# Animesh005/Torus-FHE

Measured on AMD Instinct MI355X. Metric: bootstrapped gates/sec (NAND, N=1024), higher is better.
Workload: dtype f64

## Files before the change

### torus-fhe_amd/csrc/thfhe_common.h

```cpp
#ifndef THFHE_COMMON_H
#define THFHE_COMMON_H

#include <hip/hip_runtime.h>

#include <type_traits>

#include "../../include/thfhe_hip.h"
#include "thfhe_lane.h"

namespace thfhe {

constexpr int kOpIdentity = 100;

int thfhe_fail(int code, const char *msg);
int thfhe_fail_hip(hipError_t e, const char *what);

inline int ilog2(int x) {
    int l = 0;
    while ((1 << l) < x) l++;
    return l;
}

inline int lut_validate(const thfhe_lut_spec *sp, const void *tv, int n_luts, const int32_t *lut_index, const int32_t *in0, const int32_t *in1,
                        const int32_t *in2, const int32_t *out, size_t count, int max_luts = 1024) {
// ... 5 lines not shown
    if (count > (size_t)INT32_MAX / 16) return thfhe_fail(THFHE_E_INVALID, "count too large");
    if (lut_index)
        for (size_t g = 0; g < count; g++)
            if (lut_index[g] < 0 || lut_index[g] >= n_luts) return thfhe_fail(THFHE_E_INVALID, "lut_index out of range (0 .. n_luts-1)");
    return THFHE_OK;
}

inline int lut_spec_check(const thfhe_lut_spec &sp) {
    if (sp.n_inputs < 1 || sp.n_inputs > 3) return thfhe_fail(THFHE_E_INVALID, "lut spec: n_inputs must be 1, 2 or 3");
    if (sp.theta != 1 && sp.theta != 2 && sp.theta != 4) return thfhe_fail(THFHE_E_INVALID, "lut spec: theta must be 1, 2 or 4");
    return THFHE_OK;
}

#define THFHE_HIP(expr)                                                    \
    do {                                                                   \
        hipError_t thfhe_e_ = (expr);                                      \
        if (thfhe_e_ != hipSuccess) return ::thfhe::thfhe_fail_hip(thfhe_e_, #expr); \
    } while (0)

template <int Max, int V = 1, class F>
int with_static_int(int v, const char *unsupported, F &&f) {
    if constexpr (V > Max) return thfhe_fail(THFHE_E_UNSUPPORTED, unsupported);
    else if (v == V) {
        f(std::integral_constant<int, V>{});
        return THFHE_OK;
    } else return with_static_int<Max, V + 1>(v, unsupported, f);
}
constexpr const char *kBadL = "decomposition length l must be 1..4";

inline int kernel_name_result(int len, int need) {
    return need < len ? THFHE_OK : thfhe_fail(THFHE_E_INVALID, "buffer too short for the kernel name");
}

#if defined(__HIPCC__)
#ifdef THFHE_STAMPS
#define THFHE_STAMP_STORAGE __device__ unsigned long long g_stamps[8 * 2048 * 8];
#define STAMP_DECL unsigned long long st_acc[6] = {0, 0, 0, 0, 0, 0}, st_t = __builtin_amdgcn_s_memtime()
#define STAMP(slot)                                              \
    do {                                                         \
        unsigned long long now_ = __builtin_amdgcn_s_memtime();  \
        st_acc[slot] += now_ - st_t;                             \
        st_t = now_;                                             \
    } while (0)
#define STAMP_FLUSH(wg, wave)                                                                                  \
    do {                                                                                                       \
        if (lane == 0 && (wg) < 2048)                                                                          \
            for (int q_ = 0; q_ < 6; q_++) g_stamps[(((size_t)(wg)) * 8 + (wave)) * 8 + q_] = st_acc[q_];       \
    } while (0)
#else
#define THFHE_STAMP_STORAGE
#define STAMP_DECL
#define STAMP(slot)
#define STAMP_FLUSH(wg, wave)
#endif


__device__ __forceinline__ void wave_sync() {
    __builtin_amdgcn_fence(__ATOMIC_RELEASE, "wavefront", "local");
    __builtin_amdgcn_wave_barrier();
    __builtin_amdgcn_fence(__ATOMIC_ACQUIRE, "wavefront", "local");
}

__device__ __forceinline__ int opaque_lane(int lane) {
    asm volatile("" : "+v"(lane));
    return lane;
}
typedef const int32_t __attribute__((address_space(4))) *uniform_i32_ptr;
__device__ __forceinline__ uniform_i32_ptr as_uniform(const int32_t *p) { return (uniform_i32_ptr)(size_t)p; }

template <int IMM = 0>
__device__ __forceinline__ void ring_dma(uint64_t gbase_uniform, uint32_t lane_byte_off, uint32_t lds_byte_off) {
    static_assert(IMM >= 0 && IMM < 4096, "immediate offset of a global instruction");
    asm volatile("s_nop 0\n\tglobal_load_lds_dwordx4 %0, %1 offset:%3" ::"v"(lane_byte_off), "s"(gbase_uniform), "{m0}"(lds_byte_off), "n"(IMM) : "memory");
}
template <int VM>
__device__ __forceinline__ void ring_barrier() {
    asm volatile("s_waitcnt vmcnt(%0) lgkmcnt(0)\n\ts_barrier" ::"n"(VM) : "memory");
}
__device__ __forceinline__ void wave_fft_fwd_s(int lane, cplx (&z)[8], cplx *xb, const cplx *T1, const W64 &w) {
    wave_sync();
    fwds_seg1(lane, z, xb, T1);
    wave_sync();
    fwds_seg2_ld(lane, z, xb);
    fwds_seg2_st(lane, z, xb, w);
    wave_sync();
    fwds_seg3(lane, z, xb);
}
__device__ __forceinline__ void wave_fft_inv_s(int lane, cplx (&z)[8], cplx *xb, const cplx *T1, const W64 &w) {
    wave_sync();
    invs_seg1(lane, z, xb, w);
    wave_sync();
    invs_seg2_ld(lane, z, xb);
    invs_seg2_st(lane, z, xb);
    wave_sync();
    invs_seg3(lane, z, xb, T1);
}
template <bool KEEP64 = false>
__device__ __forceinline__ void wave_transpose_hi3(cplx (&z)[8]) {
    uint32_t w[8][4];
#pragma unroll
    for (int r = 0; r < 8; r++) __builtin_memcpy(w[r], &z[r], 16);
#pragma unroll
    for (int d = 0; d < 4; d++) {
#pragma unroll
        for (int r = 0; r < 4; r++) {
            auto q = __builtin_amdgcn_permlane32_swap(w[r][d], w[r + 4][d], false, false);
            w[r][d] = q[0];
            w[r + 4][d] = q[1];
        }
#pragma unroll
        for (int r = 0; r < 8; r++) {
            if (r & 2) continue;
            auto q = __builtin_amdgcn_permlane16_swap(w[r][d], w[r + 2][d], false, false);
            w[r][d] = q[0];
            w[r + 2][d] = q[1];
        }
        if constexpr (!KEEP64) {
#pragma unroll
            for (int r = 0; r < 8; r += 2) {
                const uint32_t a = w[r][d], b = w[r + 1][d];
                w[r + 1][d] = __builtin_amdgcn_update_dpp(b, a, 0x128, 0xF, 0x3, false);
                w[r][d] = __builtin_amdgcn_update_dpp(a, b, 0x128, 0xF, 0xC, false);
            }
        }
    }
    if constexpr (KEEP64) {
#pragma unroll
        for (int r = 0; r < 8; r += 2) {
#pragma unroll
            for (int k = 0; k < 2; k++) {
                uint64_t keep = (uint64_t)w[r + 1][2 * k] | (uint64_t)w[r + 1][2 * k + 1] << 32;
                asm("" : "+v"(keep));
#pragma unroll
                for (int h = 0; h < 2; h++) {
                    const int d = 2 * k + h;
                    const uint32_t a = w[r][d], b = w[r + 1][d], kept = (uint32_t)(keep >> (32 * h));
                    w[r + 1][d] = __builtin_amdgcn_update_dpp(b, a, 0x128, 0xF, 0x3, false);
                    w[r][d] = __builtin_amdgcn_update_dpp(a, kept, 0x128, 0xF, 0xC, false);
                }
            }
        }
    }
#pragma unroll
    for (int r = 0; r < 8; r++) __builtin_memcpy(&z[r], w[r], 16);
}
__device__ __forceinline__ void wave_fft_fwd_q(int lane, cplx (&z)[8], cplx *xb, const LaneRoots &r, const W64 &w) {
    fwdq_seg1(z, r);
    wave_transpose_hi3(z);
    wave_sync();
    fwdr_seg2_st(lane, z, xb, w);
    wave_sync();
    fwd_seg3(lane, z, xb);
}
__device__ __forceinline__ void wave_fft_fwd_f(int lane, cplx (&z)[8], cplx *xb, const LaneRootsF &r) {
    fwdf_seg1(z);
    wave_transpose_hi3<true>(z);
    wave_sync();
    fwdf_seg2_st(lane, z, xb, r);
    wave_sync();
    fwdf_seg3(lane, z, xb, r);
}
template <bool LEAN>
__device__ __forceinline__ void wave_fft_inv_f(int lane, cplx (&z)[8], cplx *xb, W64 &w, LaneRoots &r, const cplx (&bc)[4]) {
    if (LEAN) opaque_in_place(w.w1), opaque_in_place(r.s);
    wave_sync();
    invf_seg1(lane, z, xb);
    wave_sync();
    inv_seg2_ld(lane, z, xb);
    invf_seg2(z, w);
    wave_transpose_hi3<true>(z);
    invf_seg3(z, r, bc);
}
__device__ __forceinline__ void wave_fft_fwd_qs(int lane, cplx (&z)[8], cplx *xb, const LaneRoots &r, const W64 &w) {
    fwdq_seg1(z, r);
    wave_transpose_hi3(z);
    wave_sync();
    fwds_seg2_st(lane, z, xb, w);
    wave_sync();
    fwds_seg3(lane, z, xb);
}
__device__ __forceinline__ void wave_fft_inv_qs(int lane, cplx (&z)[8], cplx *xb, const LaneRoots &r, const W64 &w) {
    wave_sync();
    invs_seg1(lane, z, xb, w);
    wave_sync();
    invs_seg2_ld(lane, z, xb);
    dft8<-1>(z);
    wave_transpose_hi3(z);
    invq_seg3(z, r);
}
template <int T>
__device__ __forceinline__ void wave_fft_fwd_t(int lane, cplx (&z)[8], cplx *xb, const cplx *T1t, const W64 &w) {
    wave_sync();
    fwdt_seg1<T>(lane, z, xb, T1t);
    wave_sync();
    fwds_seg2_ld(lane, z, xb);
    fwds_seg2_st(lane, z, xb, w);
    wave_sync();
    fwds_seg3(lane, z, xb);
}
template <int T>
__device__ __forceinline__ void wave_fft_inv_t(int lane, cplx (&z)[8], cplx *xb, const cplx *T1t, const W64 &w) {
    wave_sync();
    invs_seg1(lane, z, xb, w);
    wave_sync();
    invs_seg2_ld(lane, z, xb);
    invs_seg2_st(lane, z, xb);
    wave_sync();
    invt_seg3<T>(lane, z, xb, T1t);
}
template <int T, int DEN = 32>
__device__ __forceinline__ void wave_fft_fwd_tq(int lane, cplx (&z)[8], cplx *xb, const LaneRoots &r, const W64 &w) {
    fwdtq_seg1<T, DEN>(z, r);
    wave_transpose_hi3(z);
    wave_sync();
    fwds_seg2_st(lane, z, xb, w);
    wave_sync();
    fwds_seg3(lane, z, xb);
}
template <int T, int DEN = 32>
__device__ __forceinline__ void wave_fft_inv_tq(int lane, cplx (&z)[8], cplx *xb, const LaneRoots &r, const W64 &w) {
    wave_sync();
    invs_seg1(lane, z, xb, w);
    wave_sync();
    invs_seg2_ld(lane, z, xb);
    dft8<-1>(z);
    wave_transpose_hi3(z);
    invtq_seg3<T, DEN>(z, r);
}

template <int TA, int TB, int DEN = 32>
__device__ __forceinline__ void wave_fft_fwd_tq_two(int lane, cplx (&za)[8], cplx (&zb)[8], cplx *xa, cplx *xb, const LaneRoots &ra, const LaneRoots &rb,
                                                    const W64 &w) {
    fwdtq_seg1<TA, DEN>(za, ra);
    fwdtq_seg1<TB, DEN>(zb, rb);
    wave_transpose_hi3(za);
    wave_transpose_hi3(zb);
    wave_sync();
    fwds_seg2_st(lane, za, xa, w);
    fwds_seg2_st(lane, zb, xb, w);
    wave_sync();
    fwds_seg3(lane, za, xa);
    fwds_seg3(lane, zb, xb);
}
template <int TA, int TB, int DEN = 32>
__device__ __forceinline__ void wave_fft_inv_tq_two(int lane, cplx (&za)[8], cplx (&zb)[8], cplx *xb, const LaneRoots &ra, const LaneRoots &rb, const W64 &w) {
    wave_sync();
    invs_seg1(lane, za, xb, w);
    wave_sync();
    invs_seg2_ld(lane, za, xb);
    wave_sync();
    invs_seg1(lane, zb, xb, w);
    wave_sync();
    dft8<-1>(za);
    wave_transpose_hi3(za);
    invs_seg2_ld(lane, zb, xb);
    invtq_seg3<TA, DEN>(za, ra);
    dft8<-1>(zb);
    wave_transpose_hi3(zb);
    invtq_seg3<TB, DEN>(zb, rb);
}

#endif

}
#endif
```

### torus-fhe_amd/csrc/thfhe_lane.h

```cpp
#ifndef THFHE_LANE_H
#define THFHE_LANE_H

#include <limits.h>
#include <stddef.h>
#include <stdint.h>

#if defined(__HIPCC__)
#define THFHE_FN __host__ __device__ __forceinline__
#else
#define THFHE_FN inline __attribute__((always_inline))
#endif

namespace thfhe {

constexpr int kLanes = 64;
constexpr int kXbufSlots = 8 * 72;

struct alignas(16) cplx {
    double re, im;
};

THFHE_FN cplx cmul(cplx a, cplx b) { return cplx{a.re * b.re - a.im * b.im, a.re * b.im + a.im * b.re}; }
THFHE_FN cplx cmul_conj(cplx a, cplx b) {
    return cplx{a.re * b.re + a.im * b.im, a.im * b.re - a.re * b.im};
// ... 188 lines not shown
    for (int j0 = 1; j0 < 8; j0++) xbuf[xs_d(j0, lane)] = cmul_conj(z[j0], p[j0]);
}
THFHE_FN void invr_seg3(int lane, cplx (&z)[8], const cplx *xbuf, const LaneRoots &r) {
    const cplx s2 = cmul(r.s, r.s);
    cplx e = r.b, o = cmul(r.b, r.s);
#pragma unroll
    for (int k0 = 0; k0 < 8; k0 += 2) {
        z[k0] = cmul_conj(xbuf[xs_a(k0, lane)], e);
        z[k0 + 1] = cmul_conj(xbuf[xs_a(k0 + 1, lane)], o);
        if (k0 < 6) {
            e = cmul(e, s2);
            o = cmul(o, s2);
        }
    }
    dft8<-1>(z);
#pragma unroll
    for (int m = 1; m < 8; m++) z[m] = cmul_conj(z[m], cplx{THFHE_C_RE(m), THFHE_C_IM(m)});
}

THFHE_FN void fwdq_seg1(cplx (&z)[8], const LaneRoots &r) {
#pragma unroll
    for (int m = 1; m < 8; m++) z[m] = cmul(z[m], cplx{THFHE_C_RE(m), THFHE_C_IM(m)});
    dft8<+1>(z);
    const cplx s2 = cmul(r.s, r.s);
    cplx e = r.b, o = cmul(r.b, r.s);
#pragma unroll
    for (int k0 = 0; k0 < 8; k0 += 2) {
        z[k0] = cmul(z[k0], e);
        z[k0 + 1] = cmul(z[k0 + 1], o);
        if (k0 < 6) {
            e = cmul(e, s2);
            o = cmul(o, s2);
        }
    }
}
THFHE_FN void invq_seg3(cplx (&z)[8], const LaneRoots &r) {
    const cplx s2 = cmul(r.s, r.s);
    cplx e = r.b, o = cmul(r.b, r.s);
#pragma unroll
    for (int k0 = 0; k0 < 8; k0 += 2) {
        z[k0] = cmul_conj(z[k0], e);
        z[k0 + 1] = cmul_conj(z[k0 + 1], o);
        if (k0 < 6) {
            e = cmul(e, s2);
            o = cmul(o, s2);
        }
    }
    dft8<-1>(z);
#pragma unroll
    for (int m = 1; m < 8; m++) z[m] = cmul_conj(z[m], cplx{THFHE_C_RE(m), THFHE_C_IM(m)});
}

THFHE_FN cplx opaque_cplx(cplx v) {
#if defined(__HIP_DEVICE_COMPILE__)
    asm volatile("" : "+v"(v.re), "+v"(v.im));
#endif
    return v;
}
THFHE_FN void opaque_in_place(cplx &v) {
#if defined(__HIP_DEVICE_COMPILE__)
    asm volatile("" : "+v"(v.re), "+v"(v.im));
#endif
}

THFHE_FN void bfly_tw(cplx &a, cplx &b, cplx W) {
    const cplx x{__builtin_fma(-W.im, b.im, __builtin_fma(W.re, b.re, a.re)), __builtin_fma(W.im, b.re, __builtin_fma(W.re, b.im, a.im))};
    b = cplx{__builtin_fma(2.0, a.re, -x.re), __builtin_fma(2.0, a.im, -x.im)};
    a = x;
}
THFHE_FN void bfly_c4(cplx &a, cplx &b) {
    constexpr double R = 0.70710678118654752440;
    const double t = b.re - b.im, u = b.re + b.im;
    b = cplx{__builtin_fma(-R, t, a.re), __builtin_fma(-R, u, a.im)};
    a = cplx{__builtin_fma(R, t, a.re), __builtin_fma(R, u, a.im)};
}
struct RootPow {
    cplx w1, w2, w4, w1o;
};
THFHE_FN cplx csqr(cplx a) { return cplx{__builtin_fma(a.re, a.re, -(a.im * a.im)), (a.re + a.re) * a.im}; }
template <int S>
THFHE_FN RootPow root_powers(cplx w) {
    constexpr double R = 0.70710678118654752440;
    RootPow p;
    p.w1 = w;
    p.w2 = csqr(w);
    p.w4 = csqr(p.w2);
    p.w1o = S > 0 ? cplx{R * (w.re - w.im), R * (w.re + w.im)} : cplx{R * (w.re + w.im), R * (w.im - w.re)};
    return p;
}
template <int S>
THFHE_FN void dft8_tw_tail(cplx (&y)[8], cplx w1, cplx w2, cplx w1o) {
    bfly_tw(y[0], y[2], w2);
    bfly_tw(y[1], y[3], w2);
    bfly_tw(y[4], y[6], mul_si<S>(w2));
    bfly_tw(y[5], y[7], mul_si<S>(w2));
    bfly_tw(y[0], y[1], w1);
    bfly_tw(y[2], y[3], mul_si<S>(w1));
    bfly_tw(y[4], y[5], w1o);
    bfly_tw(y[6], y[7], mul_si<S>(w1o));
    const cplx x4 = y[1], x2 = y[2], x6 = y[3], x1 = y[4], x5 = y[5], x3 = y[6];
    y[1] = x1;
    y[2] = x2;
    y[3] = x3;
    y[4] = x4;
    y[5] = x5;
    y[6] = x6;
}
template <int S>
THFHE_FN void dft8_tw(cplx (&y)[8], const RootPow &p) {
#pragma unroll
    for (int m = 0; m < 4; m++) bfly_tw(y[m], y[m + 4], p.w4);
    dft8_tw_tail<S>(y, p.w1, p.w2, p.w1o);
}
THFHE_FN void dft8_tw_c32(cplx (&y)[8]) {
#pragma unroll
    for (int m = 0; m < 4; m++) bfly_c4(y[m], y[m + 4]);
    dft8_tw_tail<+1>(y, cplx{THFHE_C_RE(1), THFHE_C_IM(1)}, cplx{THFHE_C_RE(2), THFHE_C_IM(2)}, cplx{THFHE_C_RE(5), THFHE_C_IM(5)});
}
struct LaneRootsF {
    cplx s, w;
};
THFHE_FN void fwdf_seg1(cplx (&z)[8]) { dft8_tw_c32(z); }
THFHE_FN void fwdf_seg2_st(int lane, cplx (&z)[8], cplx *xbuf, const LaneRootsF &r) {
    dft8_tw<+1>(z, root_powers<+1>(r.s));
#pragma unroll
    for (int k1 = 0; k1 < 8; k1++) xbuf[xs_c(k1, lane)] = z[k1];
}
THFHE_FN void fwdf_seg3(int lane, cplx (&z)[8], const cplx *xbuf, const LaneRootsF &r) {
    fwd_seg3_ld(lane, z, xbuf);
    dft8_tw<+1>(z, root_powers<+1>(r.w));
}
THFHE_FN cplx cconj(cplx a) { return cplx{a.re, -a.im}; }
THFHE_FN void make_untwist_f(cplx b, cplx (&bc)[4]) {
    bc[0] = b;
#pragma unroll
    for (int m = 1; m < 4; m++) bc[m] = cmul(b, cplx{THFHE_C_RE(m), THFHE_C_IM(m)});
}
THFHE_FN void invf_seg1(int lane, cplx (&z)[8], cplx *xbuf) {
    dft8<-1>(z);
#pragma unroll
    for (int j0 = 0; j0 < 8; j0++) xbuf[xs_d(j0, lane)] = z[j0];
}
THFHE_FN void invf_seg2(cplx (&z)[8], const W64 &w) { dft8_tw<-1>(z, root_powers<-1>(cconj(w.w1))); }
THFHE_FN void invf_seg3(cplx (&z)[8], const LaneRoots &r, const cplx (&bc)[4]) {
    constexpr double R = 0.70710678118654752440;
    dft8_tw<-1>(z, root_powers<-1>(cconj(r.s)));
#pragma unroll
    for (int m = 0; m < 4; m++) {
        z[m] = cmul_conj(z[m], bc[m]);
        z[m + 4] = cmul_conj(cplx{R * (z[m + 4].re + z[m + 4].im), R * (z[m + 4].im - z[m + 4].re)}, bc[m]);
    }
}

THFHE_FN uint32_t rot_minus_self32(const int32_t *p, int q, int a2n, int N) {
    int e = (q - a2n) & (2 * N - 1);
    uint32_t r = (uint32_t)p[e & (N - 1)];
    if (e & N) r = 0u - r;
    return r - (uint32_t)p[q];
}
THFHE_FN double digit32(uint32_t v, int shift, uint32_t mask, int32_t half) {
    return (double)((int32_t)((v >> shift) & mask) - half);
}
THFHE_FN uint32_t decomp_offset32(int l, int Bgbit) {
    uint32_t off = 0;
    for (int p = 1; p <= l; p++) off += (1u << (Bgbit - 1)) << (32 - p * Bgbit);
    return off;
}
THFHE_FN uint32_t round_lo32(double x) {
    double y = x + 6755399441055744.0;
    uint64_t b;
    __builtin_memcpy(&b, &y, 8);
    return (uint32_t)b;
}
THFHE_FN void split_limbs32(int32_t v, double &lo, double &hi) {
    int32_t l = (int32_t)(int16_t)(uint16_t)v;
    int32_t h = (int32_t)(((int64_t)v - l) >> 16);
    lo = (double)l;
    hi = (double)h;
}

THFHE_FN int32_t modswitch2n(int32_t x, int log2_2n) {
    int32_t y = (int32_t)((uint32_t)x + (1u << (32 - log2_2n - 1)));
    return y >> (32 - log2_2n);
}


THFHE_FN size_t bk_spec_index(int i, int r, int c, int h, int rows) {
    return ((((size_t)i * rows + r) * 2 + c) * 2 + h) * 512;
}

THFHE_FN void load_rotated16(int lane, const int32_t *acc_poly, int a2n, uint32_t offset, uint32_t (&t)[16]) {
    uint32_t r[16], s[16];
#pragma unroll
    for (int m = 0; m < 16; m++) {
        const int e = (lane + 64 * m - a2n) & 2047;
        r[m] = (uint32_t)acc_poly[e & 1023];
        s[m] = (uint32_t)acc_poly[lane + 64 * m];
    }
#if defined(__HIP_DEVICE_COMPILE__)
    __builtin_amdgcn_sched_barrier(0);
#endif
#pragma unroll
    for (int m = 0; m < 16; m++) {
        const int e = (lane + 64 * m - a2n) & 2047;
        t[m] = ((e & 1024) ? 0u - r[m] : r[m]) - s[m] + offset;
    }
}
THFHE_FN void digits_to_z(const uint32_t (&t)[16], int p, int Bgbit, cplx (&z)[8]) {
    const int shift = 32 - p * Bgbit;
    const uint32_t mask = (1u << Bgbit) - 1u;
    const int32_t half = 1 << (Bgbit - 1);
#pragma unroll
    for (int m = 0; m < 8; m++) z[m] = cplx{digit32(t[m], shift, mask, half), digit32(t[m + 8], shift, mask, half)};
}
THFHE_FN int32_t sbfe32(uint32_t v, int shift, int width) {
#if defined(__HIP_DEVICE_COMPILE__)
    return __builtin_amdgcn_sbfe((int32_t)v, (uint32_t)shift, (uint32_t)width);
#else
    return (int32_t)(v << (32 - shift - width)) >> (32 - width);
#endif
}
THFHE_FN void rotated_digits_z(int lane, const int32_t *p, int a2n, int level, int l, int Bgbit, cplx (&z)[8]) {
    const int shift = 32 - level * Bgbit;
    const uint32_t off = decomp_offset32(l, Bgbit) + ((1u << (Bgbit - 1)) << shift);
    const uint32_t e4 = ((uint32_t)(lane - a2n) & 2047u) << 2;
#if defined(__HIP_DEVICE_COMPILE__)
    const uint32_t base = (uint32_t)(size_t)(__attribute__((address_space(3))) const void *)p;
#endif
    uint32_t r[8][2], s[8][2];
#pragma unroll
    for (int m = 0; m < 8; m++) {
#pragma unroll
        for (int q = 0; q < 2; q++) {
            const int c = lane + 64 * m + 512 * q;
            const uint32_t f = e4 + (uint32_t)(256 * m + 2048 * q);
#if defined(__HIP_DEVICE_COMPILE__)
            r[m][q] = (uint32_t) * (__attribute__((address_space(3))) const int32_t *)(size_t)(base | (f & 0xFFCu));
#else
            r[m][q] = (uint32_t)p[(f & 0xFFCu) >> 2];
#endif
            s[m][q] = (uint32_t)p[c];
        }
    }
#if defined(__HIP_DEVICE_COMPILE__)
    __builtin_amdgcn_sched_barrier(0);
#endif
#pragma unroll
    for (int m = 0; m < 8; m++) {
        double d[2];
#pragma unroll
        for (int q = 0; q < 2; q++) {
            const uint32_t f = e4 + (uint32_t)(256 * m + 2048 * q);
            const uint32_t M = (uint32_t)sbfe32(f, 12, 1);
            const uint32_t v = ((r[m][q] + M) ^ M) + (off - s[m][q]);
            d[q] = (double)sbfe32(v, shift, Bgbit);
        }
        z[m] = cplx{d[0], d[1]};
    }
}
THFHE_FN void diff_digits_z(int lane, const int32_t *p1, const int32_t *p0, int level, int l, int Bgbit, cplx (&z)[8]) {
    const int shift = 32 - level * Bgbit;
    const uint32_t off = decomp_offset32(l, Bgbit) + ((1u << (Bgbit - 1)) << shift);
    uint32_t r[8][2], s[8][2];
#pragma unroll
    for (int m = 0; m < 8; m++) {
#pragma unroll
        for (int q = 0; q < 2; q++) {
            const int c = lane + 64 * m + 512 * q;
            r[m][q] = (uint32_t)p1[c];
            s[m][q] = (uint32_t)p0[c];
        }
    }
#if defined(__HIP_DEVICE_COMPILE__)
    __builtin_amdgcn_sched_barrier(0);
#endif
#pragma unroll
    for (int m = 0; m < 8; m++) {
        double d[2];
#pragma unroll
        for (int q = 0; q < 2; q++) d[q] = (double)sbfe32(r[m][q] + (off - s[m][q]), shift, Bgbit);
        z[m] = cplx{d[0], d[1]};
    }
}
THFHE_FN uint32_t rotated_word(int lane, const int32_t *p, uint32_t e4, int j, uint32_t off) {
    const uint32_t f = e4 + (uint32_t)(256 * j);
#if defined(__HIP_DEVICE_COMPILE__)
    const uint32_t base = (uint32_t)(size_t)(__attribute__((address_space(3))) const void *)p;
    const uint32_t r = (uint32_t) * (__attribute__((address_space(3))) const int32_t *)(size_t)(base | (f & 0xFFCu));
#else
    const uint32_t r = (uint32_t)p[(f & 0xFFCu) >> 2];
#endif
    const uint32_t M = (uint32_t)sbfe32(f, 12, 1);
    return ((r + M) ^ M) + (off - (uint32_t)p[lane + 64 * j]);
}
template <int NF, bool BATCH = false>
THFHE_FN void rotated_fields_keep(int lane, const int32_t *p, int a2n, int l, int Bgbit, uint32_t (&t)[NF]) {
    const uint32_t off = decomp_offset32(l, Bgbit);
    const uint32_t e4 = ((uint32_t)(lane - a2n) & 2047u) << 2;
    if (!BATCH) {
#pragma unroll
        for (int j = 0; j < NF; j++) t[j] = rotated_word(lane, p, e4, j, off) ^ off;
        return;
    }
    uint32_t r[NF], s[NF];
#pragma unroll
    for (int j = 0; j < NF; j++) {
// ... 544 lines not shown
```

### torus-fhe_amd/csrc/thfhe_sk.hip

```cpp
#include <hip/hip_runtime.h>

#include <algorithm>
#include <memory>
#include <mutex>
#include <new>
#include <string>
#include <vector>

#include "../../include/thfhe_hip.h"
#include "thfhe_cb.h"
#include "thfhe_common.h"
#include "thfhe_dag.h"
#include "thfhe_devctx.h"
#include "thfhe_keyswitch.h"
#include "thfhe_lane.h"
#include "thfhe_launch_plan.h"
#include "thfhe_pack.h"
#include "thfhe_pbs_host.h"
#include "thfhe_ring_schedule.h"

using namespace thfhe;

namespace {

#include "thfhe_transform.h"

struct Lin {
    int32_t cb, cx, cy;
    int ysel;
};
__host__ __device__ inline bool gate_lin(int op, int which, Lin &L) {
    const int32_t E8 = 1 << 29, E4 = 1 << 30;
    switch (op) {
    case THFHE_NAND: L = Lin{E8, -1, -1, 1}; return true;
    case THFHE_OR: L = Lin{E8, 1, 1, 1}; return true;
    case THFHE_AND: L = Lin{-E8, 1, 1, 1}; return true;
    case THFHE_XOR: L = Lin{E4, 2, 2, 1}; return true;
    case THFHE_XNOR: L = Lin{-E4, -2, -2, 1}; return true;
    case THFHE_NOR: L = Lin{-E8, -1, -1, 1}; return true;
    case THFHE_ANDNY: L = Lin{-E8, -1, 1, 1}; return true;
    case THFHE_ANDYN: L = Lin{-E8, 1, -1, 1}; return true;
    case THFHE_ORNY: L = Lin{E8, -1, 1, 1}; return true;
    case THFHE_ORYN: L = Lin{E8, 1, -1, 1}; return true;
    case THFHE_MUX: L = which == 0 ? Lin{-E8, 1, 1, 1} : Lin{-E8, -1, 1, 2}; return true;
    case kOpIdentity: L = Lin{0, 1, 0, 1}; return true;
    default: return false;
    }
}

__global__ __launch_bounds__(256) void sk_prologue_kernel(const int32_t *__restrict__ in0, const int32_t *__restrict__ in1,
                                                           const int32_t *__restrict__ in2, int op, const int32_t *__restrict__ ops,
                                                           int rot_per_gate, int n, int n_pad, int log2_2n, long jobs,
                                                           int32_t *__restrict__ bara, int32_t *__restrict__ barb) {
    const long job = blockIdx.y;
    const int i = blockIdx.x * 256 + threadIdx.x;
    if (job >= jobs || i > n) return;
    const long gate = job / rot_per_gate;
    const int which = (int)(job % rot_per_gate);
    Lin L;
    gate_lin(ops ? ops[gate] : op, which, L);
    const size_t off = (size_t)gate * (n + 1) + i;
    uint32_t v = (uint32_t)L.cx * (uint32_t)in0[off];
    if (L.cy != 0) v += (uint32_t)L.cy * (uint32_t)(L.ysel == 2 ? in2[off] : in1[off]);
    if (i == n) {
        v += (uint32_t)L.cb;
        barb[job] = modswitch2n((int32_t)v, log2_2n);
    } else {
        bara[job * n_pad + i] = modswitch2n((int32_t)v, log2_2n);
    }
}

THFHE_STAMP_STORAGE

struct BRArgs {
    const cplx *bk;
    const cplx *tw;
    const int32_t *bara;
    const int32_t *barb;
    int32_t *out;
    long jobs;
    int n, n_pad, Bgbit;
    int32_t mu;
    const int32_t *tv;
    const int32_t *lut_idx;
    int theta;
    const int32_t *tv_a;
    const int32_t *mv_w;
    int mv_p, mv_box;
};

constexpr int kGate = 0, kLut = 1, kLutEnc = 2, kLutMv = 3;

template <int L, int W = 8, int LUT = kGate>
__global__ __launch_bounds__(64 * W, W == 8 ? 2 : 1) void sk_blind_rotate_ring_kernel(BRArgs a) {
    __shared__ __attribute__((aligned(4096))) int32_t sAcc[W][2048];
    __shared__ cplx sX[W][kXbufSlots];
    __shared__ cplx sRing[3][512];
    constexpr int ROWS = 2 * L;
    constexpr int DPC = 8 / W;
    namespace RS = ring_schedule;
    const int wave = __builtin_amdgcn_readfirstlane(threadIdx.x >> 6);
    const int lane = threadIdx.x & 63;
    W64 w64{a.tw[TwRing1k::T2 + 1 * 8 + (lane & 7)]};
    LaneRoots roots{a.tw[TwRing1k::ROOTS + 2 * lane], a.tw[TwRing1k::ROOTS + 2 * lane + 1]};
    LaneRootsF rootsf{a.tw[TwRing1k::ROOTSF + 2 * lane], a.tw[TwRing1k::ROOTSF + 2 * lane + 1]};
    const long job = (long)blockIdx.x * W + wave;
    const bool has_job = job < a.jobs;
    int32_t *acc = sAcc[wave];
    cplx *xb = sX[wave];
    const uniform_i32_ptr bara = as_uniform(a.bara + (has_job ? job : 0) * a.n_pad);
    const int Bgbit = a.Bgbit;
    if (has_job) {
        if constexpr (LUT == kLutEnc) {
            const size_t t = a.lut_idx ? (size_t)a.lut_idx[job] * 1024 : 0;
            acc_init_tlwe16(lane, acc, acc + 1024, a.barb[job], a.tv_a + t, a.tv + t);
        } else if constexpr (LUT == kLutMv) acc_init_tv16(lane, acc, acc + 1024, a.barb[job], a.tv);
        else if constexpr (LUT) acc_init_tv16(lane, acc, acc + 1024, a.barb[job], a.tv + (a.lut_idx ? (size_t)a.lut_idx[job] * 1024 : 0));
        else acc_init16(lane, acc, acc + 1024, a.barb[job], a.mu);
    }

    static_assert(DPC == 1 || DPC == 2, "a wave brings one slice of a chunk, or two 1 KiB apart");
    const uint32_t lane_off = (uint32_t)(wave * (64 * DPC) + lane) * (uint32_t)sizeof(cplx);
    uint64_t gbase = (uint64_t)(size_t)a.bk;
    int chunks_ahead = a.n * ROWS * RS::kChunksPerRow - 1;
    asm volatile("" : "+s"(gbase), "+s"(chunks_ahead));
    static_assert(RS::kResidentSlots * RS::kSlotBytes == sizeof(sRing) && RS::kSlotBytes <= sizeof(sX[0]), "ring schedule against the LDS layout");
    const uint32_t ring_base = (uint32_t)(size_t)(__attribute__((address_space(3))) void *)&sRing[0][0] + (uint32_t)wave * (1024u * DPC);
    const uint32_t lent_base = (uint32_t)(size_t)(__attribute__((address_space(3))) void *)&sX[0][0] + (uint32_t)wave * (1024u * DPC);
    auto issue = [&](int slot) {
        const uint32_t dst = slot == RS::kBorrowedSlot ? lent_base : ring_base + (uint32_t)slot * (uint32_t)RS::kSlotBytes;
        ring_dma(gbase, lane_off, dst);
        if constexpr (DPC == 2) ring_dma<1024>(gbase, lane_off, dst);
        gbase += chunks_ahead > 0 ? (uint32_t)RS::kSlotBytes : 0u;
        chunks_ahead = chunks_ahead > 0 ? chunks_ahead - 1 : 0;
    };
    auto slot_ptr = [&](int slot) -> const cplx * { return slot == RS::kBorrowedSlot ? &sX[0][0] : &sRing[slot][0]; };
    __syncthreads();
#pragma unroll
    for (int k = 0; k < RS::kPrologueIssues; k++) issue(RS::kPlan[k].slot);
    STAMP_DECL;

    for (int i = 0; i < a.n; i++) {
        const int ai = bara[i];
        const bool active = has_job && ai != 0;
        const int a2n = ai & 2047;
        cplx S[2][2][8];
#pragma unroll
        for (int c = 0; c < 2; c++)
#pragma unroll
            for (int h = 0; h < 2; h++)
#pragma unroll
                for (int m = 0; m < 8; m++) S[c][h][m] = cplx{0.0, 0.0};
        constexpr int NF = 16;
        uint32_t fld[NF];
#pragma unroll
        for (int r = 0; r < ROWS; r++) {
            cplx z[8];
            if (active) {
                int a2n_r = a2n;
                asm volatile("" : "+s"(a2n_r));
                if (r % L == 0) rotated_fields_keep<NF, W == 4>(lane, acc + (r / L) * 1024, a2n_r, L, Bgbit, fld);
                asm volatile("" : "+s"(a2n_r));
                mixed_digits_z<NF>(lane, acc + (r / L) * 1024, a2n_r, (r % L) + 1, L, Bgbit, fld, z);
                if (W == 8) opaque_in_place(rootsf.s), opaque_in_place(rootsf.w);
                wave_fft_fwd_f(lane, z, xb, rootsf);
            }
            STAMP(0);
            cplx bA[4], bB[4];
            auto consume = [&](int c4) {
                const cplx *B = slot_ptr(RS::kPlan[c4].slot);
                if (active) {
#pragma unroll
                    for (int m = 0; m < 4; m++) bA[m] = B[m * 64 + lane];
                    if (c4 > 0) {
#pragma unroll
                        for (int m = 0; m < 4; m++) cfma_negkey(S[(c4 - 1) >> 1][(c4 - 1) & 1][4 + m], z[4 + m], bB[m]);
                    }
#pragma unroll
                    for (int m = 0; m < 4; m++) bB[m] = B[(4 + m) * 64 + lane];
#pragma unroll
                    for (int m = 0; m < 4; m++) cfma_negkey(S[c4 >> 1][c4 & 1][m], z[m], bA[m]);
                }
            };
            ring_barrier<RS::vmcnt_at(RS::kBarA) * DPC>();
            STAMP(1);
#pragma unroll
            for (int k = 0; k < RS::issues_at(RS::kBarA); k++) issue(RS::issue_slot(RS::kBarA, k));
#pragma unroll
            for (int c4 = RS::first_consumed(RS::kBarA); c4 < RS::first_consumed(RS::kBarX); c4++) consume(c4);
            STAMP(2);
            ring_barrier<RS::vmcnt_at(RS::kBarX) * DPC>();
            STAMP(1);
#pragma unroll
            for (int k = 0; k < RS::issues_at(RS::kBarX); k++) issue(RS::issue_slot(RS::kBarX, k));
#pragma unroll
            for (int c4 = RS::first_consumed(RS::kBarX); c4 < RS::first_consumed(RS::kBarB); c4++) consume(c4);
            STAMP(2);
            ring_barrier<RS::vmcnt_at(RS::kBarB) * DPC>();
            static_assert(RS::issues_at(RS::kBarB) == 0 && RS::first_consumed(RS::kBarB) == RS::kChunksPerRow, "nothing is issued or read after barrier B");
            STAMP(1);
            if (active) {
#pragma unroll
                for (int m = 0; m < 4; m++) cfma_negkey(S[1][1][4 + m], z[4 + m], bB[m]);
            }
            STAMP(2);
        }
        if (active) {
            wave_sync();
            cplx bc[4];
            if (W == 8) opaque_in_place(roots.b);
            make_untwist_f(roots.b, bc);
#pragma unroll
            for (int c = 0; c < 2; c++) {
                wave_fft_inv_f<W == 8>(lane, S[c][0], xb, w64, roots, bc);
                wave_fft_inv_f<W == 8>(lane, S[c][1], xb, w64, roots, bc);
                acc_update16(lane, acc + c * 1024, S[c][0], S[c][1]);
            }
            wave_sync();
        }
        STAMP(3);
    }
    STAMP_FLUSH(blockIdx.x, wave);
    asm volatile("s_waitcnt vmcnt(0)" ::: "memory");
    if (has_job) {
        if constexpr (LUT == kLutMv) {
            const uniform_i32_ptr w = as_uniform(a.mv_w) + (size_t)(a.lut_idx ? as_uniform(a.lut_idx)[job] : 0) * a.theta * a.mv_p;
            for (int j = 0; j < a.theta; j++) extract_mv16(lane, acc, acc + 1024, w + j * a.mv_p, a.mv_p, a.mv_box, a.out + (job * a.theta + j) * 1025);
        } else if constexpr (LUT) {
            for (int j = 0; j < a.theta; j++) extract_at16(lane, acc, acc + 1024, j, a.out + (job * a.theta + j) * 1025);
        } else {
            extract16(lane, acc, acc + 1024, a.out + job * 1025);
        }
    }
}

__device__ __forceinline__ void wg_barrier() { asm volatile("s_waitcnt lgkmcnt(0)\n\ts_barrier" ::: "memory"); }
__device__ __forceinline__ void pin() { asm volatile("" ::: "memory"); }

template <int L, int LUT = kGate>
__global__ __launch_bounds__(512, 2) void sk_blind_rotate_coop_kernel(BRArgs a) {
    constexpr int ROWS = 2 * L;
    __shared__ __attribute__((aligned(4096))) int32_t sAcc[2048];
    __shared__ cplx sSpec[ROWS][512];
    __shared__ cplx sX[8][kXbufSlots];
    const int wave = __builtin_amdgcn_readfirstlane(threadIdx.x >> 6);
    const int lane = threadIdx.x & 63;
    const W64 w64{a.tw[TwRing1k::T2 + 1 * 8 + (lane & 7)]};
    const LaneRoots roots{a.tw[TwRing1k::ROOTS + 2 * lane], a.tw[TwRing1k::ROOTS + 2 * lane + 1]};
    const long job = blockIdx.x;
    const uniform_i32_ptr bara = as_uniform(a.bara + job * a.n_pad);
    const int Bgbit = a.Bgbit;
    if (wave == 0) {
        if constexpr (LUT == kLutEnc) {
            const size_t t = a.lut_idx ? (size_t)a.lut_idx[job] * 1024 : 0;
            acc_init_tlwe16(lane, sAcc, sAcc + 1024, a.barb[job], a.tv_a + t, a.tv + t);
        } else if constexpr (LUT == kLutMv) acc_init_tv16(lane, sAcc, sAcc + 1024, a.barb[job], a.tv);
        else if constexpr (LUT) acc_init_tv16(lane, sAcc, sAcc + 1024, a.barb[job], a.tv + (a.lut_idx ? (size_t)a.lut_idx[job] * 1024 : 0));
        else acc_init16(lane, sAcc, sAcc + 1024, a.barb[job], a.mu);
    }
    const int c = (wave >> 1) & 1, h = wave & 1, half = wave >> 2, r0 = half * L;
    unsigned int *ap = reinterpret_cast<unsigned int *>(sAcc) + c * 1024;
    cplx *xb = sX[wave];

    int i = 0;
    while (i < a.n && bara[i] == 0) i++;
    cplx B[L][8];
    if (i < a.n) {
#pragma unroll
        for (int r = 0; r < L; r++) load8(lane, B[r], a.bk + bk_spec_index(i, r0 + r, c, h, ROWS));
    }
    wg_barrier();
    STAMP_DECL;
    while (i < a.n) {
        const int a2n = bara[i] & 2047;
        int inext = i + 1;
        while (inext < a.n && bara[inext] == 0) inext++;
        const int inl = inext < a.n ? inext : i;
        if (wave < ROWS) {
            cplx z[8];
            rotated_digits_z(lane, sAcc + (wave / L) * 1024, a2n, (wave % L) + 1, L, Bgbit, z);
            wave_fft_fwd_q(lane, z, xb, roots, w64);
#pragma unroll
            for (int m = 0; m < 8; m++) sSpec[wave][m * 64 + lane] = z[m];
        }
        STAMP(0);
        wg_barrier();
        STAMP(1);
        cplx S[8];
#pragma unroll
        for (int m = 0; m < 8; m++) S[m] = cplx{0.0, 0.0};
#pragma unroll
        for (int r = 0; r < L; r++) {
            cplx z[8];
#pragma unroll
            for (int m = 0; m < 8; m++) z[m] = sSpec[r0 + r][m * 64 + lane];
            mac8r(S, z, B[r]);
            pin();
        }
        STAMP(2);
        if (half == 1) {
#pragma unroll
            for (int m = 0; m < 8; m++) xb[m * 64 + lane] = S[m];
            pin();
            STAMP(3);
            wg_barrier();
            STAMP(4);
#pragma unroll
            for (int r = 0; r < L; r++) {
                const cplx *src = a.bk + bk_spec_index(inl, r0 + r, c, h, ROWS);
#pragma unroll
                for (int m = 0; m < 8; m++) {
                    B[r][m] = src[m * 64 + lane];
                    pin();
                    __builtin_amdgcn_s_sleep(1);
                }
            }
        } else {
            load8(lane, B[0], a.bk + bk_spec_index(inl, r0, c, h, ROWS));
            pin();
            STAMP(3);
            wg_barrier();
            STAMP(4);
            const cplx *px = sX[wave + 4];
#pragma unroll
            for (int m = 0; m < 8; m++) {
                const cplx v = px[m * 64 + lane];
                S[m].re += v.re;
                S[m].im += v.im;
            }
            wave_sync();
            invr_seg1(lane, S, xb, w64);
            pin();
            if (L > 1) load8(lane, B[L > 1 ? 1 : 0], a.bk + bk_spec_index(inl, r0 + 1, c, h, ROWS));
            pin();
            wave_sync();
            inv_seg2_ld(lane, S, xb);
            dft8<-1>(S);
            pin();
            if (L > 2) load8(lane, B[L > 2 ? 2 : 0], a.bk + bk_spec_index(inl, r0 + 2, c, h, ROWS));
            if (L > 3) load8(lane, B[L > 3 ? 3 : 0], a.bk + bk_spec_index(inl, r0 + 3, c, h, ROWS));
            pin();
            wave_transpose_hi3(S);
            invq_seg3(S, roots);
#pragma unroll
            for (int m = 0; m < 8; m++) {
                const int q = lane + 64 * m;
                atomicAdd(ap + q, round_lo32(S[m].re) << (16 * h));
                atomicAdd(ap + q + 512, round_lo32(S[m].im) << (16 * h));
            }
        }
        STAMP(3);
        wg_barrier();
        STAMP(5);
        i = inext;
    }
    STAMP_FLUSH(blockIdx.x, wave);
    if constexpr (LUT == kLutMv) {
        const uniform_i32_ptr w = as_uniform(a.mv_w) + (size_t)(a.lut_idx ? as_uniform(a.lut_idx)[job] : 0) * a.theta * a.mv_p;
        for (int j = wave; j < a.theta; j += 8)
            extract_mv16(lane, sAcc, sAcc + 1024, w + j * a.mv_p, a.mv_p, a.mv_box, a.out + (job * a.theta + j) * 1025);
    } else if constexpr (LUT) {
        if (wave < a.theta) extract_at16(lane, sAcc, sAcc + 1024, wave, a.out + (job * a.theta + wave) * 1025);
    } else {
        if (wave == 0) extract16(lane, sAcc, sAcc + 1024, a.out + job * 1025);
    }
}

__global__ __launch_bounds__(256) void sk_linear_kernel(const int32_t *__restrict__ in0, int32_t *__restrict__ out, size_t words, int negate) {
    const size_t q = (size_t)blockIdx.x * 256 + threadIdx.x;
// ... 814 lines not shown
```

Measured before the change: 145,200.

## Use permlane-swap transpose with permuted lane order in ring FFTs

Replaces the hi3 DPP-based wave transpose in the forward and inverse fused FFTs with a new transpose that uses permlane32/permlane16 swaps. Lanes now carry a permuted frequency index (nu), so twiddles, roots, key-slot reads and the accumulator update are remapped per lane, with sign flips folded into the twiddles and untwist factors. The aim is to cut cross-lane shuffle instructions in the hot FFT path of blind rotation. In exchange it adds per-lane remapping and sign-flip logic and a nontrivial ordering that must stay bit-consistent with the key layout.

```diff
diff --git a/torus-fhe_amd/csrc/thfhe_common.h b/torus-fhe_amd/csrc/thfhe_common.h
--- a/torus-fhe_amd/csrc/thfhe_common.h
+++ b/torus-fhe_amd/csrc/thfhe_common.h
@@ -181,24 +181,70 @@
     wave_sync();
     fwd_seg3(lane, z, xb);
 }
-__device__ __forceinline__ void wave_fft_fwd_f(int lane, cplx (&z)[8], cplx *xb, const LaneRootsF &r) {
+template <bool FLIPPED>
+__device__ __forceinline__ void wave_transpose_x3(cplx (&z)[8]) {
+    uint32_t w[8][4];
+#pragma unroll
+    for (int r = 0; r < 8; r++) __builtin_memcpy(w[r], &z[r], 16);
+    if constexpr (FLIPPED) {
+#pragma unroll
+        for (int r = 4; r < 8; r++)
+#pragma unroll
+            for (int d = 0; d < 4; d++) w[r][d] = __builtin_amdgcn_update_dpp(w[r][d], w[r][d], 0x128, 0xF, 0xF, false);
+    } else {
+#pragma unroll
+        for (int r = 0; r < 4; r++) {
+#pragma unroll
+            for (int k = 0; k < 2; k++) {
+                uint64_t keep = (uint64_t)w[r + 4][2 * k] | (uint64_t)w[r + 4][2 * k + 1] << 32;
+                asm("" : "+v"(keep));
+#pragma unroll
+                for (int h = 0; h < 2; h++) {
+                    const int d = 2 * k + h;
+                    const uint32_t a = w[r][d], b = w[r + 4][d], kept = (uint32_t)(keep >> (32 * h));
+                    w[r + 4][d] = __builtin_amdgcn_update_dpp(b, a, 0x128, 0xF, 0x3, false);
+                    w[r][d] = __builtin_amdgcn_update_dpp(a, kept, 0x128, 0xF, 0xC, false);
+                }
+            }
+        }
+    }
+#pragma unroll
+    for (int d = 0; d < 4; d++) {
+#pragma unroll
+        for (int r = 0; r < 8; r++) {
+            if (r & 2) continue;
+            auto q = __builtin_amdgcn_permlane32_swap(w[r][d], w[r + 2][d], false, false);
+            w[r][d] = q[0];
+            w[r + 2][d] = q[1];
+        }
+#pragma unroll
+        for (int r = 0; r < 8; r += 2) {
+            auto q = __builtin_amdgcn_permlane16_swap(w[r][d], w[r + 1][d], false, false);
+            w[r][d] = q[0];
+            w[r + 1][d] = q[1];
+        }
+    }
+#pragma unroll
+    for (int r = 0; r < 8; r++) __builtin_memcpy(&z[r], w[r], 16);
+}
+__device__ __forceinline__ void wave_fft_fwd_x(int lane, cplx (&z)[8], cplx *xb, const LaneRootsF &r) {
     fwdf_seg1(z);
-    wave_transpose_hi3<true>(z);
-    wave_sync();
-    fwdf_seg2_st(lane, z, xb, r);
+    wave_transpose_x3<false>(z);
+    wave_sync();
+    fwdx_seg2_st(lane, z, xb, r);
     wave_sync();
     fwdf_seg3(lane, z, xb, r);
 }
 template <bool LEAN>
-__device__ __forceinline__ void wave_fft_inv_f(int lane, cplx (&z)[8], cplx *xb, W64 &w, LaneRoots &r, const cplx (&bc)[4]) {
+__device__ __forceinline__ void wave_fft_inv_x(int lane, cplx (&z)[8], cplx *xb, W64 &w, LaneRoots &r, uint32_t flip, const cplx (&bc)[4]) {
     if (LEAN) opaque_in_place(w.w1), opaque_in_place(r.s);
     wave_sync();
     invf_seg1(lane, z, xb);
     wave_sync();
     inv_seg2_ld(lane, z, xb);
     invf_seg2(z, w);
-    wave_transpose_hi3<true>(z);
-    invf_seg3(z, r, bc);
+    wave_transpose_x3<true>(z);
+    invx_seg3(z, r, flip, bc);
 }
 __device__ __forceinline__ void wave_fft_fwd_qs(int lane, cplx (&z)[8], cplx *xb, const LaneRoots &r, const W64 &w) {
     fwdq_seg1(z, r);
diff --git a/torus-fhe_amd/csrc/thfhe_lane.h b/torus-fhe_amd/csrc/thfhe_lane.h
--- a/torus-fhe_amd/csrc/thfhe_lane.h
+++ b/torus-fhe_amd/csrc/thfhe_lane.h
@@ -364,6 +364,47 @@
     }
 }
 
+THFHE_FN int lane_nu(int lane) { return (lane & 7) | ((lane & 8) << 2) | ((lane & 0x30) >> 1); }
+THFHE_FN uint32_t lane_flip_x(int lane) { return (lane & 8) ? 0x80000000u : 0u; }
+THFHE_FN double flip_sign(double v, uint32_t flip) {
+    uint64_t b;
+    __builtin_memcpy(&b, &v, 8);
+    b ^= (uint64_t)flip << 32;
+    __builtin_memcpy(&v, &b, 8);
+    return v;
+}
+THFHE_FN W64 lane_w64_x(cplx w64_j0, uint32_t flip) { return W64{cplx{flip_sign(w64_j0.re, flip), flip_sign(w64_j0.im, flip)}}; }
+template <typename WPtr>
+THFHE_FN LaneRoots lane_roots_x(const WPtr tw, int t1_base, int roots_base, int lane) {
+    const int nu = lane_nu(lane);
+    return LaneRoots{(lane & 8) ? tw[t1_base + 4 * 64 + nu] : tw[roots_base + 2 * nu], tw[roots_base + 2 * nu + 1]};
+}
+THFHE_FN void make_untwist_x(cplx b, uint32_t flip, cplx (&bc)[4]) {
+    make_untwist_f(b, bc);
+    bc[1] = cplx{flip_sign(bc[1].re, flip), flip_sign(bc[1].im, flip)};
+    bc[3] = cplx{flip_sign(bc[3].re, flip), flip_sign(bc[3].im, flip)};
+}
+THFHE_FN constexpr int fwdx_phys(int j1) { return ((j1 & 1) << 2) | ((j1 >> 2) & 1) << 1 | ((j1 >> 1) & 1); }
+THFHE_FN void fwdx_seg2_st(int lane, cplx (&z)[8], cplx *xbuf, const LaneRootsF &r) {
+    cplx y[8];
+#pragma unroll
+    for (int j1 = 0; j1 < 8; j1++) y[j1] = z[fwdx_phys(j1)];
+    dft8_tw<+1>(y, root_powers<+1>(r.s));
+#pragma unroll
+    for (int k1 = 0; k1 < 8; k1++) xbuf[xs_c(k1, lane)] = y[k1];
+}
+THFHE_FN void invx_seg3(cplx (&z)[8], const LaneRoots &r, uint32_t flip, const cplx (&bc)[4]) {
+    constexpr double R = 0.70710678118654752440;
+    RootPow p = root_powers<-1>(cconj(r.s));
+    p.w4.im = flip_sign(p.w4.im, flip);
+    dft8_tw<-1>(z, p);
+#pragma unroll
+    for (int m = 0; m < 4; m++) {
+        z[m] = cmul_conj(z[m], bc[m]);
+        z[m + 4] = cmul_conj(cplx{R * (z[m + 4].re + z[m + 4].im), R * (z[m + 4].im - z[m + 4].re)}, bc[m]);
+    }
+}
+
 THFHE_FN uint32_t rot_minus_self32(const int32_t *p, int q, int a2n, int N) {
     int e = (q - a2n) & (2 * N - 1);
     uint32_t r = (uint32_t)p[e & (N - 1)];
diff --git a/torus-fhe_amd/csrc/thfhe_sk.hip b/torus-fhe_amd/csrc/thfhe_sk.hip
--- a/torus-fhe_amd/csrc/thfhe_sk.hip
+++ b/torus-fhe_amd/csrc/thfhe_sk.hip
@@ -101,9 +101,11 @@
     namespace RS = ring_schedule;
     const int wave = __builtin_amdgcn_readfirstlane(threadIdx.x >> 6);
     const int lane = threadIdx.x & 63;
-    W64 w64{a.tw[TwRing1k::T2 + 1 * 8 + (lane & 7)]};
-    LaneRoots roots{a.tw[TwRing1k::ROOTS + 2 * lane], a.tw[TwRing1k::ROOTS + 2 * lane + 1]};
-    LaneRootsF rootsf{a.tw[TwRing1k::ROOTSF + 2 * lane], a.tw[TwRing1k::ROOTSF + 2 * lane + 1]};
+    const int nu = lane_nu(lane);
+    const uint32_t flip = lane_flip_x(lane);
+    W64 w64 = lane_w64_x(a.tw[TwRing1k::T2 + 1 * 8 + (lane & 7)], flip);
+    LaneRoots roots = lane_roots_x(a.tw, TwRing1k::T1, TwRing1k::ROOTS, lane);
+    LaneRootsF rootsf{a.tw[TwRing1k::ROOTSF + 2 * nu], a.tw[TwRing1k::ROOTSF + 2 * nu + 1]};
     const long job = (long)blockIdx.x * W + wave;
     const bool has_job = job < a.jobs;
     int32_t *acc = sAcc[wave];
@@ -163,7 +165,7 @@
                 asm volatile("" : "+s"(a2n_r));
                 mixed_digits_z<NF>(lane, acc + (r / L) * 1024, a2n_r, (r % L) + 1, L, Bgbit, fld, z);
                 if (W == 8) opaque_in_place(rootsf.s), opaque_in_place(rootsf.w);
-                wave_fft_fwd_f(lane, z, xb, rootsf);
+                wave_fft_fwd_x(lane, z, xb, rootsf);
             }
             STAMP(0);
             cplx bA[4], bB[4];
@@ -171,13 +173,13 @@
                 const cplx *B = slot_ptr(RS::kPlan[c4].slot);
                 if (active) {
 #pragma unroll
-                    for (int m = 0; m < 4; m++) bA[m] = B[m * 64 + lane];
+                    for (int m = 0; m < 4; m++) bA[m] = B[m * 64 + nu];
                     if (c4 > 0) {
 #pragma unroll
                         for (int m = 0; m < 4; m++) cfma_negkey(S[(c4 - 1) >> 1][(c4 - 1) & 1][4 + m], z[4 + m], bB[m]);
                     }
 #pragma unroll
-                    for (int m = 0; m < 4; m++) bB[m] = B[(4 + m) * 64 + lane];
+                    for (int m = 0; m < 4; m++) bB[m] = B[(4 + m) * 64 + nu];
 #pragma unroll
                     for (int m = 0; m < 4; m++) cfma_negkey(S[c4 >> 1][c4 & 1][m], z[m], bA[m]);
                 }
@@ -209,12 +211,12 @@
             wave_sync();
             cplx bc[4];
             if (W == 8) opaque_in_place(roots.b);
-            make_untwist_f(roots.b, bc);
+            make_untwist_x(roots.b, flip, bc);
 #pragma unroll
             for (int c = 0; c < 2; c++) {
-                wave_fft_inv_f<W == 8>(lane, S[c][0], xb, w64, roots, bc);
-                wave_fft_inv_f<W == 8>(lane, S[c][1], xb, w64, roots, bc);
-                acc_update16(lane, acc + c * 1024, S[c][0], S[c][1]);
+                wave_fft_inv_x<W == 8>(lane, S[c][0], xb, w64, roots, flip, bc);
+                wave_fft_inv_x<W == 8>(lane, S[c][1], xb, w64, roots, flip, bc);
+                acc_update16(nu, acc + c * 1024, S[c][0], S[c][1]);
             }
             wave_sync();
         }
```

Result: faster. 147,500 (median of 6 runs) (+1.6%).
